# caesar-one/audio-classification-using-a-deep-cnn-combined-with-multi-level-attention

Measured on AMD Instinct MI355X. Metric: 0.96 s clips/sec wave->logits (VGGish+attn), higher is better.
Workload: dtype bf16; 1 GPU; BASELINE config 3: wave->logits forward, 1024 bags x 10 s 16 kHz PCM per GPU = 10240 x 0.96 s clips per step, VGGish + MLA [2,1], random-init portable-seeded weights; f32 front-end/head, bf16 conv+FC; bags_per_gpu=1024, parallelism=dp1 (no collective: independent bags)

## Files before the change

### audio-classification-using-a-deep-cnn-combined-with-multi-level-attention_amd/csrc/conv.hip

```cpp
#include <cstdlib>
#include <type_traits>

#include "common.h"
#include "conv1_core.h"
#include "mma_core.h"

namespace {

using namespace mma;

constexpr int kThreads = 512, kWaves = 8, kMS = 6;

#ifndef MLA_CONV_STAMPS
#define MLA_CONV_STAMPS 0
#endif
#ifndef MLA_STAMP_TAP
#define MLA_STAMP_TAP 4
#define MLA_STAMP_CHUNK 5
#endif
#if MLA_CONV_STAMPS
__device__ unsigned long long g_conv_stamps[8][2][8];
#define MLA_STAMP(k) do { if (stamp_on) stamps[k] = __builtin_amdgcn_s_memtime(); } while (0)
#if MLA_CONV_STAMPS == 2
#undef MLA_STAMP
#define MLA_STAMP(k) do { } while (0)
#define MLA_STAMP2(k) do { if (stamp_on) stamps[k] = __builtin_amdgcn_s_memtime(); } while (0)
#endif
#else
#define MLA_STAMP(k) do { } while (0)
#endif

#ifndef MLA_CONV_PRIO
#define MLA_CONV_PRIO 3
#endif
#ifndef MLA_CONV_DGRAD2
#define MLA_CONV_DGRAD2 2
#endif
#ifndef MLA_CONV_NARROW_PERSIST
#define MLA_CONV_NARROW_PERSIST 0
#endif
#ifndef MLA_CONV1_RAW_BARRIER
#define MLA_CONV1_RAW_BARRIER 1
#endif
#ifndef MLA_CONV1_WAVES
#define MLA_CONV1_WAVES 3
#endif
#ifndef MLA_CONV1_ROWS
#define MLA_CONV1_ROWS 16
#endif
#ifndef MLA_CONV1_GATHER
#define MLA_CONV1_GATHER 0
#endif
#ifndef MLA_CONV_TALL
#define MLA_CONV_TALL 2
#endif
#ifndef MLA_CONV_PATCH_SPREAD
#define MLA_CONV_PATCH_SPREAD 1
#endif
#ifndef MLA_CONV_TALL_SPLIT
#define MLA_CONV_TALL_SPLIT 1
#endif
#ifndef MLA_CONV_NT_STORE
#define MLA_CONV_NT_STORE 1
#endif
#ifndef MLA_CONV_DMA_DIV
#define MLA_CONV_DMA_DIV 1
#endif
#ifndef MLA_CONV_DMA_LATE
#define MLA_CONV_DMA_LATE 1
#endif
#ifndef MLA_CONV_STAGGER
#define MLA_CONV_STAGGER 1
#endif

template <typename T, int CIN_, int COUT_, int H_, int W_, bool POOL_, int NS_, bool ACT_ = true, bool SPLIT_ = false, int WM_ = 2>
struct Cfg {
    static constexpr int WM = WM_, WN = kWaves / WM_;
    using elem = T;
    static constexpr int CIN = CIN_, COUT = COUT_, H = H_, W = W_, NS = NS_;
    static constexpr bool POOL = POOL_;
    static constexpr bool ACT = ACT_;
    static constexpr bool SPLIT = SPLIT_;
    static constexpr int CIN_A = SPLIT ? 2 * CIN : CIN;
    static constexpr int CIN_W = SPLIT ? 3 * CIN : CIN;
    static constexpr int COUT_MEM = SPLIT ? 2 * COUT : COUT;
    static_assert(!SPLIT || (sizeof(T) == 2 && ACT_), "the split mode is a bf16 forward mode");
    static constexpr int SEGW = W >= 16 ? 16 : 8;
    static constexpr int SEGS = W / SEGW;
    static constexpr int IMGS = SEGW == 8 ? WM : 1;
    static constexpr int TH = SEGW == 8 ? 12 : kMS * WM / SEGS;
    static constexpr int PW = (W == 8 && WM == 4) ? 9 : W + 2, PH = TH + 2;
    static constexpr int BN = WN * NS * 16;
    static constexpr int KC = Elem<T>::kPerRow;
    static constexpr int A_PIX = IMGS * PH * PW + (PW & 1);
    static constexpr int A_BYTES = (A_PIX + 7) / 8 * 8 * kRowBytes;
    static constexpr int B_BYTES = BN * kRowBytes;
    static constexpr int TILES_Y = H / TH;
    static constexpr bool PERSIST = NS > 2 || SPLIT || (MLA_CONV_NARROW_PERSIST && sizeof(T) == 2 && NS == 2 && POOL_ && ACT_) ||
                                    (MLA_CONV_DGRAD2 == 2 && sizeof(T) == 2 && NS == 2 && WM_ == 4 && !ACT_ && COUT_ == 64);
    static constexpr int MIN_WAVES = (PERSIST || sizeof(T) == 4) ? 2 : 4;
    static constexpr bool A_DMA = PERSIST;
    static constexpr int A_BUFS = A_DMA ? 2 : 1;
    static constexpr bool PATCH_SPREAD = MLA_CONV_PATCH_SPREAD && WM_ == 4 && CIN_ >= 256;
    static constexpr bool STAGGER = PERSIST && MLA_CONV_STAGGER;
    static constexpr int LDS_BYTES = A_BUFS * A_BYTES + 2 * B_BYTES;
    static constexpr int HO = POOL ? H / 2 : H, WO = POOL ? W / 2 : W;
    static_assert(W == 32 || W == 16 || W == 8, "tile mapping covers the VGGish widths");
    static_assert(WM == 2 || WM == 4, "waves are laid out 2 x 4 or 4 x 2");
    static_assert(H % TH == 0 && CIN % KC == 0 && COUT % BN == 0, "shape must tile exactly");
    static_assert((PW * kRowBytes) % 256 == 0 || (W == 8 && (PH * PW) % 2 == 0), "row pitch / image distance must keep the bank swizzle invariant");
    static_assert(LDS_BYTES <= 160 * 1024, "tile does not fit LDS");
};

template <typename T, int N> __device__ __forceinline__ void store_vec(T* p, const float* v);
template <> __device__ __forceinline__ void store_vec<float, 4>(float* p, const float* v) {
    *reinterpret_cast<f32x4*>(p) = f32x4{v[0], v[1], v[2], v[3]};
}
template <> __device__ __forceinline__ void store_vec<float, 2>(float* p, const float* v) {
    typedef float f32x2 __attribute__((ext_vector_type(2)));
    *reinterpret_cast<f32x2*>(p) = f32x2{v[0], v[1]};
}
template <> __device__ __forceinline__ void store_vec<bf16_t, 4>(bf16_t* p, const float* v) {
#if MLA_CONV_NT_STORE
    __builtin_nontemporal_store(u32x2{pack_bf16x2(v[0], v[1]), pack_bf16x2(v[2], v[3])}, reinterpret_cast<u32x2*>(p));
#else
    *reinterpret_cast<u32x2*>(p) = u32x2{pack_bf16x2(v[0], v[1]), pack_bf16x2(v[2], v[3])};
#endif
}
template <> __device__ __forceinline__ void store_vec<bf16_t, 2>(bf16_t* p, const float* v) {
    *reinterpret_cast<uint32_t*>(p) = pack_bf16x2(v[0], v[1]);
}

template <> __device__ __forceinline__ void store_vec<float, 1>(float* p, const float* v) { *p = v[0]; }
template <> __device__ __forceinline__ void store_vec<bf16_t, 1>(bf16_t* p, const float* v) { p->bits = f2bf(v[0]); }

template <typename C>
__device__ __forceinline__ void store_px(typename C::elem* p, const float* v) {
    using T = typename C::elem;
    if constexpr (C::SPLIT) {
        float hi[C::NS], lo[C::NS];
        _Pragma("unroll") for (int j = 0; j < C::NS; ++j) {
            hi[j] = bf2f(f2bf(v[j]));
            lo[j] = v[j] - hi[j];
        }
        store_vec<T, C::NS>(p, hi);
        store_vec<T, C::NS>(p + C::COUT, lo);
    } else {
        store_vec<T, C::NS>(p, v);
    }
}

template <typename C>
__device__ __forceinline__ int a_swizzle(int xh, int img) {
    (void)img;
    return ((xh >> 1) & 3) << 1;
}

template <typename C>
__global__ __launch_bounds__(kThreads, C::MIN_WAVES) void conv3x3_kernel(const typename C::elem* __restrict__ in,
                                                               const typename C::elem* __restrict__ wgt,
                                                               const float* __restrict__ bias,
                                                               typename C::elem* __restrict__ out, int n_img, int n_tiles,
                                                               typename C::elem* __restrict__ prepool, uint8_t* __restrict__ codes) {
    using T = typename C::elem;
    constexpr int PER = Elem<T>::kPerChunk;
    extern __shared__ __attribute__((aligned(16))) char smem[];
    char* sA = smem;
    char* sB = smem + C::A_BUFS * C::A_BYTES;

    const int t = threadIdx.x, lane = t & 63, wave = t >> 6, wm = wave / C::WN, wn = wave % C::WN;
    const int r = lane & 15, q = lane >> 4;
    const int ty = blockIdx.x % C::TILES_Y;
    const int y_tile = ty * C::TH;
    const int n0 = blockIdx.y * C::BN;
    int tile = blockIdx.x;
    int img0 = (tile / C::TILES_Y) * C::IMGS;

    const int wimg = C::SEGW == 8 ? 2 * (wm >> 1) : 0;
    const int wxh = C::SEGS == 2 ? (wm & 1) : 0, wy = C::SEGS == 2 ? (wm >> 1) : (C::SEGW == 8 ? (wm & 1) : wm);
    const int l_img = C::SEGW == 8 ? wimg + (r >> 3) : 0;
    const int l_x = C::SEGW == 8 ? (r & 7) : (wxh * 16 + r);
    const int l_y0 = kMS * wy;
    int abase[3];
    _Pragma("unroll") for (int kx = 0; kx < 3; ++kx) {
        const int xh = l_x + kx;
        abase[kx] = ((l_img * C::PH + l_y0) * C::PW + xh) * kRowBytes + 16 * (q ^ a_swizzle<C>(xh, l_img));
    }
    const int bbase = tile_off(wn * C::NS * 16 + r, q);

    const int nb = n0 + (wn * 16 + r) * C::NS;
    float bv[C::NS];
    _Pragma("unroll") for (int j = 0; j < C::NS; ++j) bv[j] = C::ACT ? bias[nb + j] : 0.f;
    f32x4 acc[kMS][C::NS];
    _Pragma("unroll") for (int i = 0; i < kMS; ++i)
        _Pragma("unroll") for (int j = 0; j < C::NS; ++j) acc[i][j] = f32x4{bv[j], bv[j], bv[j], bv[j]};

    constexpr int A_PIECES = C::IMGS * C::PH * C::PW * 8;
    constexpr int A_PASSES = (A_PIECES + kThreads - 1) / kThreads;
    constexpr int CHUNKS = C::CIN_W / C::KC;
    constexpr int PLANE = C::CIN / C::KC;
    auto a_chan = [](int c) { return (!C::SPLIT ? c : (c % 3 < 2 ? c / 3 : PLANE + c / 3)) * C::KC; };

    constexpr uint32_t ESZ = sizeof(T);
    auto patch_rsrc = [&](int first_img) {
        const int imgs_here = (n_img - first_img) < C::IMGS ? (n_img - first_img) : C::IMGS;
        return __builtin_amdgcn_make_buffer_rsrc(const_cast<T*>(in) + size_t(first_img) * C::H * C::W * C::CIN_A, 0,
                                                 uint32_t(imgs_here) * C::H * C::W * C::CIN_A * ESZ, 0x00020000);
    };
    __amdgpu_buffer_rsrc_t a_rsrc = patch_rsrc(img0);
    const __amdgpu_buffer_rsrc_t b_rsrc = __builtin_amdgcn_make_buffer_rsrc(
        const_cast<T*>(wgt) + size_t(n0) * 9 * C::CIN_W, 0, uint32_t(C::BN) * 9 * C::CIN_W * ESZ, 0x00020000);
    u32x4 apre[A_PASSES];
    auto a_load = [&](int c0) {
        _Pragma("unroll") for (int p = 0; p < A_PASSES; ++p) {
            const int piece = t + kThreads * p;
            const int ch = piece & 7, pix = piece >> 3;
            const int xh = pix % C::PW, rest = pix / C::PW;
            const int yh = rest % C::PH, im = rest / C::PH;
            const int gy = y_tile + yh - 1, gx = xh - 1;
            const bool ok = piece < A_PIECES && gy >= 0 && gy < C::H && gx >= 0 && gx < C::W;
            const int voff = ok ? int((((im * C::H + gy) * C::W + gx) * C::CIN_A + ch * PER) * ESZ) : int(0x7fffff00);
            apre[p] = __builtin_amdgcn_raw_buffer_load_b128(a_rsrc, voff, int(c0 * ESZ), 0);
        }
    };
    auto a_write = [&]() {
        _Pragma("unroll") for (int p = 0; p < A_PASSES; ++p) {
            const int piece = t + kThreads * p;
            const int ch = piece & 7, pix = piece >> 3;
            const int xh = pix % C::PW, rest = pix / C::PW;
            const int yh = rest % C::PH, im = rest / C::PH;
            if (piece < A_PIECES)
                lds_write16(sA, ((im * C::PH + yh) * C::PW + xh) * kRowBytes + 16 * (ch ^ a_swizzle<C>(xh, im)), apre[p]);
        }
    };
    auto b_dma = [&](int c0, int tap, int buf_off) {
        _Pragma("unroll") for (int p = 0; p < C::BN / 64 / MLA_CONV_DMA_DIV; ++p) {
            const int row = 8 * (wave + 8 * p) + (lane >> 3), slot = lane & 7;
            const int chunk = slot ^ (((row >> 1) & 3) << 1);
            const int n = (row & ~(C::NS * 16 - 1)) + (row & 15) * C::NS + ((row >> 4) & (C::NS - 1));
            __builtin_amdgcn_raw_ptr_buffer_load_lds(b_rsrc, (__attribute__((address_space(3))) void*)(sB + buf_off + 8 * (wave + 8 * p) * kRowBytes),
                                                 16, int((n * 9 * C::CIN_W + chunk * PER) * ESZ), int((tap * C::CIN_W + c0) * ESZ), 0, 0);
        }
    };

    constexpr int A_INSTRS = (C::A_PIX + 7) / 8;
    constexpr int A_ROUNDS = (A_INSTRS + 7) / 8;
    static_assert(A_ROUNDS <= 9, "a patch is staged within the nine taps of the previous chunk");
    auto a_dma_round = [&](int c0, int abuf, int p) {
        const int wi = wave + 8 * p;
        if (wi < A_INSTRS) {
            const int pix = 8 * wi + (lane >> 3), slot = lane & 7;
            const int xh = pix % C::PW, rest = pix / C::PW;
            const int yh = rest % C::PH, im = rest / C::PH;
            const int gy = y_tile + yh - 1, gx = xh - 1;
            const bool ok = pix < C::A_PIX && gy >= 0 && gy < C::H && gx >= 0 && gx < C::W;
            const int chunk = slot ^ a_swizzle<C>(xh, im);
            const int voff = ok ? int((((im * C::H + gy) * C::W + gx) * C::CIN_A + chunk * PER) * ESZ) : int(0x7fffff00);
            __builtin_amdgcn_raw_ptr_buffer_load_lds(a_rsrc, (__attribute__((address_space(3))) void*)(sA + abuf * C::A_BYTES + wi * 8 * kRowBytes),
                                                     16, voff, int(c0 * ESZ), 0, 0);
        }
    };
    auto a_dma = [&](int c0, int abuf) {
        _Pragma("unroll") for (int p = 0; p < A_ROUNDS; ++p) a_dma_round(c0, abuf, p);
    };

    int abuf = 0;
    if constexpr (C::A_DMA) {
        for (int i = t; i < C::A_BUFS * C::A_BYTES / 16; i += kThreads) lds_write16(sA, 16 * i, zero16());
        __syncthreads();
        a_dma(0, 0);
        b_dma(0, 0, 0);
    } else {
        a_load(0);
        b_dma(0, 0, 0);
        a_write();
    }
    asm volatile("s_waitcnt vmcnt(0)" ::: "memory");
    __syncthreads();

    int par = 0;
    const bool late = C::STAGGER && __builtin_amdgcn_readfirstlane(wave) >= 4;
#if MLA_CONV_PRIO == 1 || MLA_CONV_PRIO == 3
    if (C::PERSIST && __builtin_amdgcn_readfirstlane(wave) >= 4) __builtin_amdgcn_s_setprio(1);
#elif MLA_CONV_PRIO == 2
    if (C::PERSIST && __builtin_amdgcn_readfirstlane(wave) < 4) __builtin_amdgcn_s_setprio(1);
#endif
#if MLA_CONV_STAMPS
    unsigned long long stamps[8] = {0, 0, 0, 0, 0, 0, 0, 0};
    int chunk_counter = 0;
#endif
    auto run = [&](auto late_c) {
    constexpr bool LATE = decltype(late_c)::value;
    u32x4 af[kMS], bf[C::NS];
    for (;;) {
        const int next_tile = tile + int(gridDim.x);
        const bool has_next = C::PERSIST && next_tile < n_tiles;
        for (int c = 0; c < CHUNKS; ++c) {
            const int c0 = c * C::KC;
            const bool last_chunk = c + 1 == CHUNKS;
            const bool more = !last_chunk || has_next;
            const bool new_patch = more && !(C::SPLIT && !last_chunk && c % 3 == 0);
            _Pragma("unroll") for (int tap = 0; tap < 9; ++tap) {
                const int ky = tap / 3, kx = tap % 3;
                const int cur = par ? C::B_BYTES : 0;
                auto issue_dma = [&]() {
                    if (tap < 8) b_dma(c0, tap + 1, cur ^ C::B_BYTES);
                    else if (more) b_dma(last_chunk ? 0 : c0 + C::KC, 0, cur ^ C::B_BYTES);
                    if constexpr (C::A_DMA) {
                        if constexpr (C::PATCH_SPREAD) {
                          if (tap < A_ROUNDS && new_patch) {
                            if (tap == 0 && last_chunk) a_rsrc = patch_rsrc((next_tile / C::TILES_Y) * C::IMGS);
                            a_dma_round(last_chunk ? 0 : a_chan(c + 1), abuf ^ 1, tap);
                          }
                        } else if (tap == 2 && new_patch) {
                            if (last_chunk) a_rsrc = patch_rsrc((next_tile / C::TILES_Y) * C::IMGS);
                            a_dma(last_chunk ? 0 : a_chan(c + 1), abuf ^ 1);
                        }
                    } else {
                        if (tap == 5 && new_patch) {
                            if (last_chunk) a_rsrc = patch_rsrc((next_tile / C::TILES_Y) * C::IMGS);
                            a_load(last_chunk ? 0 : a_chan(c + 1));
                        }
                    }
                };
                auto rd = [&](int ks) {
                    _Pragma("unroll") for (int i = 0; i < kMS; ++i)
                        af[i] = lds_read16(sA + abuf * C::A_BYTES, (abase[kx] ^ (ks << 6)) + (i + ky) * C::PW * kRowBytes);
                    _Pragma("unroll") for (int j = 0; j < C::NS; ++j)
                        bf[j] = lds_read16(sB, cur + (bbase ^ (ks << 6)) + j * 16 * kRowBytes);
                };
                auto mm = [&]() {
                    __builtin_amdgcn_sched_barrier(0);
                    _Pragma("unroll") for (int i = 0; i < kMS; ++i)
                        _Pragma("unroll") for (int j = 0; j < C::NS; ++j) mma_step<T>(af[i], bf[j], acc[i][j]);
                    __builtin_amdgcn_sched_barrier(0);
                };
#if MLA_CONV_STAMPS == 1
                const bool stamp_on = tap == MLA_STAMP_TAP && chunk_counter == MLA_STAMP_CHUNK && (wave == 0 || wave == 4) && blockIdx.x < 8 && blockIdx.y == 0;
#endif
                if constexpr (!LATE) {
                    MLA_STAMP(0);
#if MLA_CONV_PRIO == 3
                    __builtin_amdgcn_s_setprio(2);
#endif
                    if (!MLA_CONV_DMA_LATE) issue_dma();
                    rd(0);
                    if (MLA_CONV_DMA_LATE) issue_dma();
                    MLA_STAMP(1);
#if MLA_CONV_STAMPS == 1
                    if (stamp_on) asm volatile("s_waitcnt lgkmcnt(0)" ::: "memory");
#endif
                    MLA_STAMP(2);
                    mm();
                    MLA_STAMP(3);
#if MLA_CONV_PRIO == 3
                    __builtin_amdgcn_s_setprio(0);
#endif
                    rd(1);
#if MLA_CONV_STAMPS == 1
                    if (stamp_on) asm volatile("s_waitcnt lgkmcnt(0)" ::: "memory");
#endif
                    MLA_STAMP(4);
                    mm();
                    MLA_STAMP(5);
                } else {
#if MLA_CONV_PRIO == 3
                    __builtin_amdgcn_s_setprio(3);
#endif
                    MLA_STAMP(0);
                    if (!MLA_CONV_DMA_LATE) issue_dma();
                    if (tap > 0 || c > 0) mm();
                    if (MLA_CONV_DMA_LATE) issue_dma();
                    MLA_STAMP(1);
#if MLA_CONV_PRIO == 3
                    __builtin_amdgcn_s_setprio(1);
#endif
                    rd(0);
#if MLA_CONV_STAMPS == 1
                    if (stamp_on) asm volatile("s_waitcnt lgkmcnt(0)" ::: "memory");
#endif
                    MLA_STAMP(2);
                    mm();
                    MLA_STAMP(3);
                    rd(1);
                    MLA_STAMP(4);
                    asm volatile("s_waitcnt lgkmcnt(0)" ::: "memory");
                    MLA_STAMP(5);
                }
                asm volatile("s_waitcnt vmcnt(0)" ::: "memory");
                MLA_STAMP(6);
                __syncthreads();
                MLA_STAMP(7);
#if MLA_CONV_STAMPS
                if (tap == 8) ++chunk_counter;
#endif
                if constexpr (C::A_DMA) {
                    if (tap == 8 && new_patch) abuf ^= 1;
                } else {
                    if (tap == 8 && new_patch) {
                        a_write();
                        __syncthreads();
                    }
                }
                par ^= 1;
            }
        }

#if MLA_CONV_STAMPS == 2
        const bool stamp_on = chunk_counter == MLA_STAMP_CHUNK && (wave == 0 || wave == 4) && blockIdx.x < 8 && blockIdx.y == 0;
        MLA_STAMP2(0);
#endif
        if constexpr (LATE) {
            __builtin_amdgcn_sched_barrier(0);
            _Pragma("unroll") for (int i = 0; i < kMS; ++i)
                _Pragma("unroll") for (int j = 0; j < C::NS; ++j) mma_step<T>(af[i], bf[j], acc[i][j]);
            __builtin_amdgcn_sched_barrier(0);
        }
#if MLA_CONV_STAMPS == 2
        MLA_STAMP2(1);
#endif
        {
            if (C::POOL) {
                if (!C::SPLIT && prepool) {
                    _Pragma("unroll") for (int i = 0; i < kMS; ++i) {
                        const int y = y_tile + l_y0 + i;
                        _Pragma("unroll") for (int e = 0; e < 4; ++e) {
                            float v[C::NS];
                            _Pragma("unroll") for (int j = 0; j < C::NS; ++j) v[j] = fmaxf(acc[i][j][e], 0.f);
                            const int rr = 4 * q + e;
                            const int img = img0 + (C::SEGW == 8 ? wimg + (rr >> 3) : 0);
                            const int x = C::SEGW == 8 ? (rr & 7) : ((wxh * 16) + rr);
                            if (img < n_img) store_vec<T, C::NS>(prepool + ((size_t(img) * C::H + y) * C::W + x) * C::COUT + nb, v);
                        }
                    }
                }
                _Pragma("unroll") for (int ip = 0; ip < kMS / 2; ++ip) {
                    float p0[C::NS], p1[C::NS];
                    _Pragma("unroll") for (int j = 0; j < C::NS; ++j) {
                        const f32x4 u = acc[2 * ip][j], d = acc[2 * ip + 1][j];
                        p0[j] = fmaxf(fmaxf(fmaxf(u.x, u.y), fmaxf(d.x, d.y)), 0.f);
                        p1[j] = fmaxf(fmaxf(fmaxf(u.z, u.w), fmaxf(d.z, d.w)), 0.f);
                    }
                    const int yo = (y_tile + l_y0 + 2 * ip) >> 1;
                    const int img = img0 + (C::SEGW == 8 ? wimg + (q >> 1) : 0);
                    const int xo = C::SEGW == 8 ? 2 * (q & 1) : (((wxh * 16) + 4 * q) >> 1);
                    if (img < n_img) {
                        T* o = out + ((size_t(img) * C::HO + yo) * C::WO + xo) * C::COUT_MEM + nb;
                        store_px<C>(o, p0);
                        store_px<C>(o + C::COUT_MEM, p1);
                    }
                    if constexpr (!C::SPLIT) {
                        if (codes && img < n_img) {
                            auto code_of = [](float a0, float a1, float a2, float a3) -> uint32_t {
                                const bool m1 = a1 > a0;
                                const float b1 = m1 ? a1 : a0;
                                const bool m2 = a2 > b1;
                                const float b2 = m2 ? a2 : b1;
                                const bool m3 = a3 > b2;
                                const float b3 = m3 ? a3 : b2;
                                return b3 > 0.f ? (m3 ? 3u : (m2 ? 2u : (m1 ? 1u : 0u))) : 4u;
                            };
                            uint32_t c0 = 0u, c1 = 0u;
                            _Pragma("unroll") for (int j = 0; j < C::NS; ++j) {
                                const f32x4 u = acc[2 * ip][j], d = acc[2 * ip + 1][j];
                                c0 |= code_of(u.x, u.y, d.x, d.y) << (8 * j);
                                c1 |= code_of(u.z, u.w, d.z, d.w) << (8 * j);
                            }
                            uint8_t* cp = codes + ((size_t(img) * C::HO + yo) * C::WO + xo) * C::COUT + nb;
                            if constexpr (C::NS == 4) {
                                *reinterpret_cast<uint32_t*>(cp) = c0;
                                *reinterpret_cast<uint32_t*>(cp + C::COUT) = c1;
                            } else if constexpr (C::NS == 2) {
                                *reinterpret_cast<uint16_t*>(cp) = uint16_t(c0);
                                *reinterpret_cast<uint16_t*>(cp + C::COUT) = uint16_t(c1);
                            } else {
                                cp[0] = uint8_t(c0);
                                cp[C::COUT] = uint8_t(c1);
                            }
                        }
                    }
                }
            } else {
                _Pragma("unroll") for (int i = 0; i < kMS; ++i) {
                    const int y = y_tile + l_y0 + i;
                    _Pragma("unroll") for (int e = 0; e < 4; ++e) {
                        float v[C::NS];
                        _Pragma("unroll") for (int j = 0; j < C::NS; ++j) v[j] = C::ACT ? fmaxf(acc[i][j][e], 0.f) : acc[i][j][e];
                        const int rr = 4 * q + e;
                        const int img = img0 + (C::SEGW == 8 ? wimg + (rr >> 3) : 0);
                        const int x = C::SEGW == 8 ? (rr & 7) : ((wxh * 16) + rr);
                        if (img < n_img) store_px<C>(out + ((size_t(img) * C::H + y) * C::W + x) * C::COUT_MEM + nb, v);
                    }
                }
            }
        }
#if MLA_CONV_STAMPS == 2
        MLA_STAMP2(2);
#endif
        if (!has_next) break;
        tile = next_tile;
        img0 = (tile / C::TILES_Y) * C::IMGS;
        _Pragma("unroll") for (int i = 0; i < kMS; ++i)
            _Pragma("unroll") for (int j = 0; j < C::NS; ++j) acc[i][j] = f32x4{bv[j], bv[j], bv[j], bv[j]};
    }
    };
    if constexpr (C::STAGGER) {
        if (late) run(std::true_type{});
        else run(std::false_type{});
    } else {
        run(std::false_type{});
    }
#if MLA_CONV_STAMPS
    if ((wave == 0 || wave == 4) && lane == 0 && blockIdx.x < 8 && blockIdx.y == 0)
        for (int k = 0; k < 8; ++k) g_conv_stamps[blockIdx.x][wave >> 2][k] = stamps[k];
#endif
}

template <typename T> struct Conv1Frag;
template <> struct Conv1Frag<bf16_t> { u32x4 b[4]; };
template <> struct Conv1Frag<float> { float b[3][4]; };

template <typename TIN, typename T, bool SPLIT = false>
__global__ __launch_bounds__(256, 4) void conv1_kernel(const TIN* __restrict__ x, const float* __restrict__ w,
                                                    const float* __restrict__ bias, T* __restrict__ out, int n_img) {
    constexpr int PITCH = 68;
    constexpr int ROW = 64 * int(sizeof(T)) + 16;
    __shared__ float sX[20 * PITCH];
    __shared__ __attribute__((aligned(16))) char sOut[4 * 32 * ROW];
    const int t = threadIdx.x, lane = t & 63, wave = t >> 6, r = lane & 15, q = lane >> 4;
    const int n_tiles = n_img * 12;

    float pre[3];
    auto patch_load = [&](int tile) {
        const int img = tile / 12, y0 = (tile % 12) * 8;
        _Pragma("unroll") for (int k = 0; k < 3; ++k) {
            const int p = t + 256 * k, yh = p / 66, xh = p % 66;
            const int gy = y0 + yh - 1, gx = xh - 1;
            const int cy = gy < 0 ? 0 : (gy > 95 ? 95 : gy), cx = gx < 0 ? 0 : (gx > 63 ? 63 : gx);
            const float v = load_elem<TIN>(x + (size_t(img) * 96 + cy) * 64 + cx);
            pre[k] = (p < 660 && gy >= 0 && gy < 96 && gx >= 0 && gx < 64) ? v : 0.f;
        }
    };
    auto patch_write = [&]() {
        _Pragma("unroll") for (int k = 0; k < 3; ++k) {
            const int p = t + 256 * k;
            if (p < 660) sX[(p / 66) * PITCH + p % 66] = pre[k];
        }
    };
    int tile = blockIdx.x;
    patch_load(tile);
    for (int p = t; p < 10 * PITCH; p += 256) sX[10 * PITCH + p] = 0.f;

    Conv1Frag<T> wf;
    int toff[8];
    if constexpr (sizeof(T) == 2) {
        _Pragma("unroll") for (int j = 0; j < 4; ++j) {
            uint32_t pk[4];
            _Pragma("unroll") for (int e = 0; e < 4; ++e) {
                const int t0 = 8 * q + 2 * e, t1 = t0 + 1;
                const float v0 = t0 < 9 ? w[(4 * r + j) * 9 + t0] : 0.f, v1 = t1 < 9 ? w[(4 * r + j) * 9 + t1] : 0.f;
                pk[e] = pack_bf16x2(v0, v1);
            }
            wf.b[j] = u32x4{pk[0], pk[1], pk[2], pk[3]};
        }
        _Pragma("unroll") for (int e = 0; e < 8; ++e) {
            const int tt = 8 * q + e;
            toff[e] = tt < 9 ? (tt / 3) * PITCH + tt % 3 + r : 10 * PITCH;
        }
    } else {
        _Pragma("unroll") for (int s3 = 0; s3 < 3; ++s3) {
            const int tt = 4 * s3 + q;
            _Pragma("unroll") for (int j = 0; j < 4; ++j) wf.b[s3][j] = tt < 9 ? w[(4 * r + j) * 9 + tt] : 0.f;
            toff[s3] = tt < 9 ? (tt / 3) * PITCH + tt % 3 + r : 10 * PITCH;
        }
    }
    float bj[4];
    _Pragma("unroll") for (int j = 0; j < 4; ++j) bj[j] = bias[4 * r + j];

    char* stage = sOut + wave * 32 * ROW;
    for (; tile < n_tiles; tile += gridDim.x) {
    const int img = tile / 12, y0 = (tile % 12) * 8;
    patch_write();
    __syncthreads();
    if (tile + int(gridDim.x) < n_tiles) patch_load(tile + int(gridDim.x));
    _Pragma("unroll") for (int seg = 0; seg < 4; ++seg) {
        f32x4 acc[2][4];
        _Pragma("unroll") for (int i = 0; i < 2; ++i)
            _Pragma("unroll") for (int j = 0; j < 4; ++j) acc[i][j] = f32x4{0.f, 0.f, 0.f, 0.f};
        _Pragma("unroll") for (int i = 0; i < 2; ++i) {
            const int shift = (2 * wave + i) * PITCH + 16 * seg;
            if constexpr (sizeof(T) == 2) {
                float v[8];
                _Pragma("unroll") for (int e = 0; e < 8; ++e) v[e] = sX[toff[e] + shift];
                const u32x4 a = u32x4{pack_bf16x2(v[0], v[1]), pack_bf16x2(v[2], v[3]), pack_bf16x2(v[4], v[5]), pack_bf16x2(v[6], v[7])};
                _Pragma("unroll") for (int j = 0; j < 4; ++j) mma_step<bf16_t>(a, wf.b[j], acc[i][j]);
            } else {
                _Pragma("unroll") for (int s3 = 0; s3 < 3; ++s3) {
                    const float a = sX[toff[s3] + shift];
                    _Pragma("unroll") for (int j = 0; j < 4; ++j)
                        acc[i][j] = __builtin_amdgcn_mfma_f32_16x16x4f32(a, wf.b[s3][j], acc[i][j], 0, 0, 0);
                }
            }
        }
        {
            float p0[4], p1[4];
            _Pragma("unroll") for (int j = 0; j < 4; ++j) {
                const f32x4 u = acc[0][j], d = acc[1][j];
                p0[j] = fmaxf(fmaxf(fmaxf(u.x, u.y), fmaxf(d.x, d.y)) + bj[j], 0.f);
                p1[j] = fmaxf(fmaxf(fmaxf(u.z, u.w), fmaxf(d.z, d.w)) + bj[j], 0.f);
            }
            const int xo = 8 * seg + 2 * q;
            if constexpr (SPLIT) {
                static_assert(!SPLIT || sizeof(T) == 4, "split output is produced by the exact-f32 path");
                float h0[4], h1[4], l0[4], l1[4];
                _Pragma("unroll") for (int j = 0; j < 4; ++j) {
                    h0[j] = bf2f(f2bf(p0[j])); l0[j] = p0[j] - h0[j];
                    h1[j] = bf2f(f2bf(p1[j])); l1[j] = p1[j] - h1[j];
                }
                bf16_t* s0 = reinterpret_cast<bf16_t*>(stage + xo * ROW) + 4 * r;
                bf16_t* s1 = reinterpret_cast<bf16_t*>(stage + (xo + 1) * ROW) + 4 * r;
                store_vec<bf16_t, 4>(s0, h0); store_vec<bf16_t, 4>(s0 + 64, l0);
                store_vec<bf16_t, 4>(s1, h1); store_vec<bf16_t, 4>(s1 + 64, l1);
            } else {
                store_vec<T, 4>(reinterpret_cast<T*>(stage + xo * ROW) + 4 * r, p0);
                store_vec<T, 4>(reinterpret_cast<T*>(stage + (xo + 1) * ROW) + 4 * r, p1);
            }
        }
    }
    __builtin_amdgcn_fence(__ATOMIC_RELEASE, "wavefront");
    __builtin_amdgcn_wave_barrier();
    __builtin_amdgcn_fence(__ATOMIC_ACQUIRE, "wavefront");
    constexpr int PIECES = 64 * int(sizeof(T)) / 16;
    char* dst = reinterpret_cast<char*>(out + ((size_t(img) * 48 + y0 / 2 + wave) * 32) * 64);
    _Pragma("unroll") for (int it = 0; it < PIECES / 2; ++it) {
        const int piece = it * 64 + lane, p = piece / PIECES, c = piece % PIECES;
        *reinterpret_cast<u32x4*>(dst + size_t(piece) * 16) = *reinterpret_cast<const u32x4*>(stage + p * ROW + c * 16);
    }
    __syncthreads();
    }
}

template <typename TIN>
__global__ __launch_bounds__(256, MLA_CONV1_WAVES) void conv1_patch_kernel(const TIN* __restrict__ x, const float* __restrict__ w,
                                                            const float* __restrict__ bias, bf16_t* __restrict__ out, int n_img) {
    using conv1::f32x16;
    constexpr int TR = MLA_CONV1_ROWS;
    constexpr int TPC = 96 / TR;
    constexpr int NP = (TR + 2) * 66;
    constexpr int NL = (NP + 255) / 256;
    constexpr int PITCH = conv1::kPitch;
    constexpr int ROW = conv1::kStageRow;
    __shared__ __attribute__((aligned(16))) uint16_t sX[(TR + 2) * PITCH];
    __shared__ __attribute__((aligned(16))) char sOut[4 * 32 * ROW];
    const int t = threadIdx.x, lane = t & 63, wave = t >> 6, px = lane & 31, h = lane >> 5;
    const int n_tiles = n_img * TPC;

    bf16x8 wa[4][2];
    f32x16 binit[2];
    _Pragma("unroll") for (int pos = 0; pos < 4; ++pos)
        _Pragma("unroll") for (int mt = 0; mt < 2; ++mt) wa[pos][mt] = conv1::weight_frag(w, pos, mt, lane);
    _Pragma("unroll") for (int mt = 0; mt < 2; ++mt) binit[mt] = conv1::bias_frag(bias, mt, lane);

    float pre[NL];
    auto patch_load = [&](int tile) {
        const int img = tile / TPC, y0 = (tile % TPC) * TR;
        _Pragma("unroll") for (int k = 0; k < NL; ++k) {
            const int p = t + 256 * k, yh = p / 66, xh = p % 66;
            const int gy = y0 + yh - 1, gx = xh - 1;
            const int cy = gy < 0 ? 0 : (gy > 95 ? 95 : gy), cx = gx < 0 ? 0 : (gx > 63 ? 63 : gx);
            const float v = load_elem<TIN>(x + (size_t(img) * 96 + cy) * 64 + cx);
            pre[k] = (p < NP && gy >= 0 && gy < 96 && gx >= 0 && gx < 64) ? v : 0.f;
        }
    };
    auto patch_write = [&]() {
        _Pragma("unroll") for (int k = 0; k < NL; ++k) {
            const int p = t + 256 * k;
            if (p < NP) sX[(p / 66) * PITCH + p % 66] = f2bf(pre[k]);
        }
    };
    auto lds_barrier = [&]() {
#if MLA_CONV1_RAW_BARRIER
        asm volatile("s_waitcnt lgkmcnt(0)" ::: "memory");
        __builtin_amdgcn_s_barrier();
#else
        __syncthreads();
#endif
    };
    int tile = blockIdx.x;
    if (tile < n_tiles) patch_load(tile);
    char* stage = sOut + wave * 32 * ROW;
    for (; tile < n_tiles; tile += gridDim.x) {
        const int img = tile / TPC, y0 = (tile % TPC) * TR;
        patch_write();
        lds_barrier();
        if (tile + int(gridDim.x) < n_tiles) patch_load(tile + int(gridDim.x));
        _Pragma("unroll") for (int rr = 0; rr < TR / 8; ++rr) {
            const int prow = wave * (TR / 8) + rr;
            char* gdst = reinterpret_cast<char*>(out + ((size_t(img) * 48 + y0 / 2 + prow) * 32) * 64);
            conv1::pooled_row(sX + (2 * prow) * PITCH, wa, binit, stage, gdst, lane);
        }
        lds_barrier();
    }
}

template <typename T>
__global__ void repack_kernel(const float* __restrict__ w, T* __restrict__ out, int cout, int cin) {
    const int64_t total = int64_t(cout) * 9 * cin;
    for (int64_t i = int64_t(blockIdx.x) * blockDim.x + threadIdx.x; i < total; i += int64_t(gridDim.x) * blockDim.x) {
        const int c = int(i % cin);
        const int tap = int((i / cin) % 9);
        const int o = int(i / (int64_t(cin) * 9));
        store_elem<T>(out + i, w[(int64_t(o) * cin + c) * 9 + tap]);
    }
}

template <typename T>
__global__ void repack_dgrad_kernel(const float* __restrict__ w, T* __restrict__ out, int cout, int cin) {
    const int64_t total = int64_t(cout) * 9 * cin;
    for (int64_t i = int64_t(blockIdx.x) * blockDim.x + threadIdx.x; i < total; i += int64_t(gridDim.x) * blockDim.x) {
        const int co = int(i % cout);
        const int tap = int((i / cout) % 9);
        const int ci = int(i / (int64_t(cout) * 9));
        store_elem<T>(out + i, w[(int64_t(co) * cin + ci) * 9 + (8 - tap)]);
    }
}

template <typename T>
int repack_dgrad(const float* w_oihw, int64_t cout, int64_t cin, T* out, mla_stream_t stream) {
    MLA_REQUIRE(w_oihw && out && cout > 0 && cin > 0, MLA_E_ARG, "bad repack arguments");
    const int64_t total = cout * 9 * cin;
    const unsigned grid = unsigned((total + 255) / 256 < 4096 ? (total + 255) / 256 : 4096);
    hipLaunchKernelGGL(repack_dgrad_kernel<T>, dim3(grid), dim3(256), 0, static_cast<hipStream_t>(stream), w_oihw, out, int(cout), int(cin));
    MLA_LAUNCH_OK("repack_dgrad_kernel");
    return MLA_OK;
}

template <typename T>
__global__ void convert_kernel(const float* __restrict__ in, T* __restrict__ out, int64_t n) {
    for (int64_t i = int64_t(blockIdx.x) * blockDim.x + threadIdx.x; i < n; i += int64_t(gridDim.x) * blockDim.x)
        store_elem<T>(out + i, in[i]);
}

__global__ void widen_kernel(const bf16_t* __restrict__ in, float* __restrict__ out, int64_t n) {
    for (int64_t i = int64_t(blockIdx.x) * blockDim.x + threadIdx.x; i < n; i += int64_t(gridDim.x) * blockDim.x)
        out[i] = bf2f(in[i].bits);
}

inline bool wide_tiles() {
    const char* e = getenv("MLA_CONV_TILE");
    return e && e[0] == 'w';
}

template <typename C>
int launch_conv(const void* in, const void* w, const float* bias, void* out, int64_t n_img, hipStream_t s, void* prepool = nullptr,
                uint8_t* codes = nullptr) {
    using T = typename C::elem;
    auto kern = conv3x3_kernel<C>;
    MLA_HIP_OK(hipFuncSetAttribute(reinterpret_cast<const void*>(kern), hipFuncAttributeMaxDynamicSharedMemorySize,
                                   C::LDS_BYTES));
    const int64_t tiles = ((n_img + C::IMGS - 1) / C::IMGS) * C::TILES_Y;
    MLA_REQUIRE(tiles <= 0x7fffffff, MLA_E_SHAPE, "too many tiles");
    int dev = 0, cus = 256;
    if (hipGetDevice(&dev) == hipSuccess) hipDeviceGetAttribute(&cus, hipDeviceAttributeMultiprocessorCount, dev);
    constexpr int n_tiles_n = C::COUT / C::BN;
    constexpr int per_cu = (C::LDS_BYTES * 2 <= 160 * 1024 && C::MIN_WAVES >= 4) ? 2 : 1;
    int64_t gx = int64_t(cus) * per_cu / n_tiles_n;
    gx = gx / C::TILES_Y * C::TILES_Y;
    if (gx < C::TILES_Y) gx = C::TILES_Y;
    if (gx > tiles || !C::PERSIST) gx = tiles;
    hipLaunchKernelGGL(kern, dim3(unsigned(gx), n_tiles_n), dim3(kThreads), C::LDS_BYTES, s,
                       static_cast<const T*>(in), static_cast<const T*>(w), bias, static_cast<T*>(out), int(n_img), int(tiles), static_cast<T*>(prepool), codes);
    MLA_LAUNCH_OK("conv3x3_kernel");
    return MLA_OK;
}

template <typename T>
int conv_layer(int layer, const void* in, const void* w, const float* bias, void* out, int64_t n, hipStream_t s) {
    if constexpr (sizeof(T) == 2 && MLA_CONV_TALL) {
        if (!wide_tiles()) switch (layer) {
            case 2: return launch_conv<Cfg<T, 64, 128, 48, 32, true, 4, true, false, 4>>(in, w, bias, out, n, s);
            case 3: return launch_conv<Cfg<T, 128, 256, 24, 16, false, 4, true, false, 4>>(in, w, bias, out, n, s);
            case 4: return launch_conv<Cfg<T, 256, 256, 24, 16, true, 4, true, false, 4>>(in, w, bias, out, n, s);
#if MLA_CONV_TALL >= 2
            case 5: return launch_conv<Cfg<T, 256, 512, 12, 8, false, 4, true, false, 4>>(in, w, bias, out, n, s);
            case 6: return launch_conv<Cfg<T, 512, 512, 12, 8, true, 4, true, false, 4>>(in, w, bias, out, n, s);
#endif
        }
    }
    switch (layer) {
        case 2: return launch_conv<Cfg<T, 64, 128, 48, 32, true, 2>>(in, w, bias, out, n, s);
        case 3: return launch_conv<Cfg<T, 128, 256, 24, 16, false, 4>>(in, w, bias, out, n, s);
        case 4: return launch_conv<Cfg<T, 256, 256, 24, 16, true, 4>>(in, w, bias, out, n, s);
        case 5: return launch_conv<Cfg<T, 256, 512, 12, 8, false, 4>>(in, w, bias, out, n, s);
        case 6: return launch_conv<Cfg<T, 512, 512, 12, 8, true, 4>>(in, w, bias, out, n, s);
// ... 255 lines not shown
```

Before: 859,600 clips/s.

## Prefetch next tile's first DMA before epilogue and use buffer stores with counted vmcnt waits

```diff
diff --git a/audio-classification-using-a-deep-cnn-combined-with-multi-level-attention_amd/csrc/conv.hip b/audio-classification-using-a-deep-cnn-combined-with-multi-level-attention_amd/csrc/conv.hip
--- a/audio-classification-using-a-deep-cnn-combined-with-multi-level-attention_amd/csrc/conv.hip
+++ b/audio-classification-using-a-deep-cnn-combined-with-multi-level-attention_amd/csrc/conv.hip
@@ -134,8 +134,21 @@
 template <> __device__ __forceinline__ void store_vec<float, 1>(float* p, const float* v) { *p = v[0]; }
 template <> __device__ __forceinline__ void store_vec<bf16_t, 1>(bf16_t* p, const float* v) { p->bits = f2bf(v[0]); }
 
+template <typename T, int N>
+__device__ __forceinline__ void store_vec_buf(__amdgpu_buffer_rsrc_t rs, int off, int soff, const float* v) {
+    if constexpr (sizeof(T) == 4) {
+        if constexpr (N == 4) __builtin_amdgcn_raw_buffer_store_b128(__builtin_bit_cast(u32x4, f32x4{v[0], v[1], v[2], v[3]}), rs, off, soff, 0);
+        else if constexpr (N == 2) __builtin_amdgcn_raw_buffer_store_b64(u32x2{__builtin_bit_cast(uint32_t, v[0]), __builtin_bit_cast(uint32_t, v[1])}, rs, off, soff, 0);
+        else __builtin_amdgcn_raw_buffer_store_b32(__builtin_bit_cast(uint32_t, v[0]), rs, off, soff, 0);
+    } else {
+        if constexpr (N == 4) __builtin_amdgcn_raw_buffer_store_b64(u32x2{pack_bf16x2(v[0], v[1]), pack_bf16x2(v[2], v[3])}, rs, off, soff, MLA_CONV_NT_STORE ? 2 : 0);
+        else if constexpr (N == 2) __builtin_amdgcn_raw_buffer_store_b32(pack_bf16x2(v[0], v[1]), rs, off, soff, 0);
+        else __builtin_amdgcn_raw_buffer_store_b16(f2bf(v[0]), rs, off, soff, 0);
+    }
+}
+
 template <typename C>
-__device__ __forceinline__ void store_px(typename C::elem* p, const float* v) {
+__device__ __forceinline__ void store_px(__amdgpu_buffer_rsrc_t rs, int off, int soff, const float* v) {
     using T = typename C::elem;
     if constexpr (C::SPLIT) {
         float hi[C::NS], lo[C::NS];
@@ -143,11 +156,28 @@
             hi[j] = bf2f(f2bf(v[j]));
             lo[j] = v[j] - hi[j];
         }
-        store_vec<T, C::NS>(p, hi);
-        store_vec<T, C::NS>(p + C::COUT, lo);
+        store_vec_buf<T, C::NS>(rs, off, soff, hi);
+        store_vec_buf<T, C::NS>(rs, off, soff + C::COUT * int(sizeof(T)), lo);
     } else {
-        store_vec<T, C::NS>(p, v);
-    }
+        store_vec_buf<T, C::NS>(rs, off, soff, v);
+    }
+}
+
+template <typename C>
+struct EpilogueStores {
+    static constexpr int OUT = (C::POOL ? kMS / 2 * 2 : kMS * 4) * (C::SPLIT ? 2 : 1);
+    static constexpr bool TRAIN = C::POOL && !C::SPLIT;
+    static constexpr int PREPOOL = TRAIN ? kMS * 4 : 0;
+    static constexpr int CODES = TRAIN ? kMS / 2 * 2 : 0;
+    static_assert(OUT + PREPOOL <= 63, "vmcnt is a 6-bit counter");
+};
+
+template <int N>
+__device__ __forceinline__ void wait_vmcnt_lds() {
+    static_assert(N >= 0 && N <= 63, "vmcnt is a 6-bit counter");
+    asm volatile("" ::: "memory");
+    __builtin_amdgcn_s_waitcnt((N & 15) | ((N >> 4) << 14) | (7 << 4) | (0 << 8));
+    asm volatile("" ::: "memory");
 }
 
 template <typename C>
@@ -210,6 +240,10 @@
     __amdgpu_buffer_rsrc_t a_rsrc = patch_rsrc(img0);
     const __amdgpu_buffer_rsrc_t b_rsrc = __builtin_amdgcn_make_buffer_rsrc(
         const_cast<T*>(wgt) + size_t(n0) * 9 * C::CIN_W, 0, uint32_t(C::BN) * 9 * C::CIN_W * ESZ, 0x00020000);
+    auto store_rsrc = [&](auto* base, int per_img) {
+        const int imgs_here = (n_img - img0) < C::IMGS ? (n_img - img0) : C::IMGS;
+        return __builtin_amdgcn_make_buffer_rsrc(base + size_t(img0) * per_img, 0, uint32_t(imgs_here) * per_img * uint32_t(sizeof(*base)), 0x00020000);
+    };
     u32x4 apre[A_PASSES];
     auto a_load = [&](int c0) {
         _Pragma("unroll") for (int p = 0; p < A_PASSES; ++p) {
@@ -292,6 +326,14 @@
     auto run = [&](auto late_c) {
     constexpr bool LATE = decltype(late_c)::value;
     u32x4 af[kMS], bf[C::NS];
+    bool primed = false;
+    auto first_tap_dma = [&]() {
+        b_dma(0, 1, par ? 0 : C::B_BYTES);
+        if constexpr (C::PATCH_SPREAD && !C::SPLIT) {
+            static_assert(CHUNKS > 1, "a spread patch belongs to the next chunk of the same tile");
+            a_dma_round(a_chan(1), abuf ^ 1, 0);
+        }
+    };
     for (;;) {
         const int next_tile = tile + int(gridDim.x);
         const bool has_next = C::PERSIST && next_tile < n_tiles;
@@ -303,7 +345,9 @@
             _Pragma("unroll") for (int tap = 0; tap < 9; ++tap) {
                 const int ky = tap / 3, kx = tap % 3;
                 const int cur = par ? C::B_BYTES : 0;
+                const bool ahead = C::PERSIST && tap == 0 && c == 0 && primed;
                 auto issue_dma = [&]() {
+                    if (ahead) return;
                     if (tap < 8) b_dma(c0, tap + 1, cur ^ C::B_BYTES);
                     else if (more) b_dma(last_chunk ? 0 : c0 + C::KC, 0, cur ^ C::B_BYTES);
                     if constexpr (C::A_DMA) {
@@ -387,9 +431,19 @@
                     asm volatile("s_waitcnt lgkmcnt(0)" ::: "memory");
                     MLA_STAMP(5);
                 }
-                asm volatile("s_waitcnt vmcnt(0)" ::: "memory");
-                MLA_STAMP(6);
-                __syncthreads();
+                if (ahead) {
+                    using ES = EpilogueStores<C>;
+                    if (ES::TRAIN && prepool && !codes) wait_vmcnt_lds<ES::OUT + ES::PREPOOL>();
+                    else if (ES::TRAIN && codes && !prepool) wait_vmcnt_lds<ES::OUT + ES::CODES>();
+                    else wait_vmcnt_lds<ES::OUT>();
+                    MLA_STAMP(6);
+                    __builtin_amdgcn_s_barrier();
+                    asm volatile("" ::: "memory");
+                } else {
+                    asm volatile("s_waitcnt vmcnt(0)" ::: "memory");
+                    MLA_STAMP(6);
+                    __syncthreads();
+                }
                 MLA_STAMP(7);
 #if MLA_CONV_STAMPS
                 if (tap == 8) ++chunk_counter;
@@ -419,18 +473,27 @@
 #if MLA_CONV_STAMPS == 2
         MLA_STAMP2(1);
 #endif
+        if constexpr (C::PERSIST) {
+            primed = has_next;
+            if (has_next) first_tap_dma();
+        }
         {
+            constexpr int ESB = int(sizeof(T));
+            const __amdgpu_buffer_rsrc_t o_rsrc = store_rsrc(out, C::HO * C::WO * C::COUT_MEM);
+            const int e_img = C::SEGW == 8 ? wimg + (q >> 1) : 0;
+            const int e_x = C::SEGW == 8 ? 4 * (q & 1) : wxh * 16 + 4 * q;
+            const int e_y = y_tile + l_y0;
+            int pix_full = ((e_img * C::H + e_y) * C::W + e_x);
+            int pix_pool = ((e_img * C::HO + (e_y >> 1)) * C::WO + (e_x >> 1));
+            asm volatile("" : "+v"(pix_full), "+v"(pix_pool));
             if (C::POOL) {
                 if (!C::SPLIT && prepool) {
+                    const __amdgpu_buffer_rsrc_t p_rsrc = store_rsrc(prepool, C::H * C::W * C::COUT);
                     _Pragma("unroll") for (int i = 0; i < kMS; ++i) {
-                        const int y = y_tile + l_y0 + i;
                         _Pragma("unroll") for (int e = 0; e < 4; ++e) {
                             float v[C::NS];
                             _Pragma("unroll") for (int j = 0; j < C::NS; ++j) v[j] = fmaxf(acc[i][j][e], 0.f);
-                            const int rr = 4 * q + e;
-                            const int img = img0 + (C::SEGW == 8 ? wimg + (rr >> 3) : 0);
-                            const int x = C::SEGW == 8 ? (rr & 7) : ((wxh * 16) + rr);
-                            if (img < n_img) store_vec<T, C::NS>(prepool + ((size_t(img) * C::H + y) * C::W + x) * C::COUT + nb, v);
+                            store_vec_buf<T, C::NS>(p_rsrc, (pix_full * C::COUT + nb) * ESB, (i * C::W + e) * C::COUT * ESB, v);
                         }
                     }
                 }
@@ -441,16 +504,12 @@
                         p0[j] = fmaxf(fmaxf(fmaxf(u.x, u.y), fmaxf(d.x, d.y)), 0.f);
                         p1[j] = fmaxf(fmaxf(fmaxf(u.z, u.w), fmaxf(d.z, d.w)), 0.f);
                     }
-                    const int yo = (y_tile + l_y0 + 2 * ip) >> 1;
-                    const int img = img0 + (C::SEGW == 8 ? wimg + (q >> 1) : 0);
-                    const int xo = C::SEGW == 8 ? 2 * (q & 1) : (((wxh * 16) + 4 * q) >> 1);
-                    if (img < n_img) {
-                        T* o = out + ((size_t(img) * C::HO + yo) * C::WO + xo) * C::COUT_MEM + nb;
-                        store_px<C>(o, p0);
-                        store_px<C>(o + C::COUT_MEM, p1);
-                    }
+                    const int o = (pix_pool * C::COUT_MEM + nb) * ESB;
+                    store_px<C>(o_rsrc, o, ip * C::WO * C::COUT_MEM * ESB, p0);
+                    store_px<C>(o_rsrc, o, (ip * C::WO + 1) * C::COUT_MEM * ESB, p1);
                     if constexpr (!C::SPLIT) {
-                        if (codes && img < n_img) {
+                        if (codes) {
+                            const __amdgpu_buffer_rsrc_t c_rsrc = store_rsrc(codes, C::HO * C::WO * C::COUT);
                             auto code_of = [](float a0, float a1, float a2, float a3) -> uint32_t {
                                 const bool m1 = a1 > a0;
                                 const float b1 = m1 ? a1 : a0;
@@ -466,30 +525,26 @@
                                 c0 |= code_of(u.x, u.y, d.x, d.y) << (8 * j);
                                 c1 |= code_of(u.z, u.w, d.z, d.w) << (8 * j);
                             }
-                            uint8_t* cp = codes + ((size_t(img) * C::HO + yo) * C::WO + xo) * C::COUT + nb;
+                            const int cp = pix_pool * C::COUT + nb, cs = ip * C::WO * C::COUT;
                             if constexpr (C::NS == 4) {
-                                *reinterpret_cast<uint32_t*>(cp) = c0;
-                                *reinterpret_cast<uint32_t*>(cp + C::COUT) = c1;
+                                __builtin_amdgcn_raw_buffer_store_b32(c0, c_rsrc, cp, cs, 0);
+                                __builtin_amdgcn_raw_buffer_store_b32(c1, c_rsrc, cp, cs + C::COUT, 0);
                             } else if constexpr (C::NS == 2) {
-                                *reinterpret_cast<uint16_t*>(cp) = uint16_t(c0);
-                                *reinterpret_cast<uint16_t*>(cp + C::COUT) = uint16_t(c1);
+                                __builtin_amdgcn_raw_buffer_store_b16(uint16_t(c0), c_rsrc, cp, cs, 0);
+                                __builtin_amdgcn_raw_buffer_store_b16(uint16_t(c1), c_rsrc, cp, cs + C::COUT, 0);
                             } else {
-                                cp[0] = uint8_t(c0);
-                                cp[C::COUT] = uint8_t(c1);
+                                __builtin_amdgcn_raw_buffer_store_b8(uint8_t(c0), c_rsrc, cp, cs, 0);
+                                __builtin_amdgcn_raw_buffer_store_b8(uint8_t(c1), c_rsrc, cp, cs + C::COUT, 0);
                             }
                         }
                     }
                 }
             } else {
                 _Pragma("unroll") for (int i = 0; i < kMS; ++i) {
-                    const int y = y_tile + l_y0 + i;
                     _Pragma("unroll") for (int e = 0; e < 4; ++e) {
                         float v[C::NS];
                         _Pragma("unroll") for (int j = 0; j < C::NS; ++j) v[j] = C::ACT ? fmaxf(acc[i][j][e], 0.f) : acc[i][j][e];
-                        const int rr = 4 * q + e;
-                        const int img = img0 + (C::SEGW == 8 ? wimg + (rr >> 3) : 0);
-                        const int x = C::SEGW == 8 ? (rr & 7) : ((wxh * 16) + rr);
-                        if (img < n_img) store_px<C>(out + ((size_t(img) * C::H + y) * C::W + x) * C::COUT_MEM + nb, v);
+                        store_px<C>(o_rsrc, (pix_full * C::COUT_MEM + nb) * ESB, (i * C::W + e) * C::COUT_MEM * ESB, v);
                     }
                 }
             }
```

After: 853,000 clips/s. About the same (-0.8%).
